# castorini/howl

Hardware: AMD Instinct MI355X
Metric: utterances/sec/node (res8 end-to-end training step, 1s@16kHz, 40-mel) (higher is better)
Workload: dtype f32; 1 GPU; res8 training step (frontend+fwd+xent+bwd+AdamW), 512 x 1 s utterances per GPU, 12 labels -- BASELINE configs[2] per-GPU share: res8 GSC-12, 512 x 1 s per GPU (4096 over 8); global_batch=512, samples_per_utterance=16000, labels=12, parallelism=single, frontend=eval

## Files before the change

### howl_amd/csrc/res8.hip

```cpp
#include "howl_common.hip.h"
#include "../../include/howl_hip.h"

namespace {

struct HowlPtrs6 {
    float* p[6];
};
constexpr int MAX_WINDOWS = 64;
struct HowlWinRows {
    int lo[MAX_WINDOWS], hi[MAX_WINDOWS];
};
struct HowlBnBuffers {
    float* running_mean;
    float* running_var;
    long long* num_batches;
};
struct BnFold {
    const float* part;
    int nparts;
    double count;
    float* stats_out;
    HowlBnBuffers bn;
};

// ... 631 lines not shown
#pragma unroll
                    for (int hh = 0; hh < 2; ++hh) ev[i][hh] = *reinterpret_cast<const float2*>(ebase + ea.off(i, hh));
            }
            HOWL_STAIR(1);
            k_run<NTW>(k, acc, c.CS, b2);
            k_tail<NTW>(k, acc, dl);
            HOWL_STAIR(0);
        }
        if constexpr (NTW > 0) conv_epilogue<MODE, NTW, TS, HALO>(acc, ev, epi, ubase, c.t0, lane, st0, st1, b, pv);
        __syncthreads();
    }
}

struct BwdFold {
    const float* stats;
    const float* m12;
    const float* part;
    int nparts;
    double count;
};
__device__ __forceinline__ void bwd_consts_to_lds(float* lm, int ch, float mean, float rstd, float m1, float m2) {
    lm[ch] = rstd;
    lm[CP + ch] = -rstd * rstd * m2;
    lm[2 * CP + ch] = rstd * (mean * rstd * m2 - m1);
}
__device__ __forceinline__ void bwd_fold_to_lds(float* lm, const BwdFold& f, int tid, int nthreads) {
    const int lane = tid & 63, wave = tid >> 6;
    if (f.part == nullptr) {
        if (tid < CP) bwd_consts_to_lds(lm, tid, f.stats[tid], f.stats[CP + tid], f.m12[tid], f.m12[CP + tid]);
    } else {
        const int c8 = lane >> 3;
        for (int ch0 = 4 * wave; ch0 < CP; ch0 += 4 * (nthreads >> 6)) {
            const int ch = ch0 + (c8 & 3);
            const float mean = f.stats[ch], rstd = f.stats[CP + ch];
            const double acc = fold_part_column(f.part, part_stride(f.nparts), f.nparts, (c8 < 4 ? 0 : CP) + ch, lane);
            const double second = __shfl_xor(acc, 32);
            if (c8 < 4 && (lane & 7) == 0)
                bwd_consts_to_lds(lm, ch, mean, rstd, (float)(acc / f.count), (float)(second / f.count));
        }
    }
}

struct WFold {
    const float* part;
    int nparts;
    float* out;
};

template <int MODE, int SLICES, int HALO = 0>
__device__ __forceinline__ void conv3x3_body(
    StageCfg cfg,
    const float* __restrict__ in_stats,
    const float* __restrict__ wp,
    const float* __restrict__ res,
// ... 741 lines not shown
        conv3x3_body<1, SD, HALO>(zc, nullptr, wp, nullptr, dx, xs, xs_stats, spart, nullptr, B, H, j, nblk, r, BnFold{}, bfold, wf, sg);
    else
        wgrad_body<SW, HALO>(WStage{zc, s_prev, false}, in_stats, bfold, wpart, B, H, j, nblk, r - SD, sg);
}

struct RowsAdamW {
    float* p;
    const float* g0;
    float* m;
    float* v;
    HowlAdamWCoef c;
    long rest_lo, rest_hi;
    int on;
};
__device__ __forceinline__ void reduce_rows_body(const float* __restrict__ part, int nparts, int ncols, int mode,
                                                 float* __restrict__ out, const RowsAdamW& opt) {
    __shared__ float red[16][64];
    const int lane = threadIdx.x & 63, rg = threadIdx.x >> 6, nrg = blockDim.x >> 6;
    const int col = blockIdx.x * 64 + lane;
    float s = 0.0f;
    if (col < ncols) {
        const float* src = part + col;
        for (int g = rg; g < nparts; g += 8 * nrg) {
            float v[8];
#pragma unroll
            for (int u = 0; u < 8; ++u) {
                const int r = g + u * nrg;
                v[u] = src[(size_t)(r < nparts ? r : nparts - 1) * ncols];
            }
#pragma unroll
            for (int u = 0; u < 8; ++u) s += (g + u * nrg < nparts) ? v[u] : 0.0f;
        }
    }
    red[rg][lane] = s;
    __syncthreads();
    if (rg == 0 && col < ncols) {
        float tot = red[0][lane];
        for (int r = 1; r < nrg; ++r) tot += red[r][lane];
        long d = -1;
        if (mode == 0) {
            d = col;
        } else {
            const int co = col / WNCOL, idx = col - co * WNCOL;
            if (co < NMAP && idx < WTAPS) d = (co * NMAP + idx % NMAP) * 9 + idx / NMAP;
        }
        if (d >= 0) {
            out[d] = tot;
            if (opt.on) howl_adamw_element(opt.p, opt.m, opt.v, (size_t)((out - opt.g0) + d), tot, opt.c);
        }
    }
}

__global__ __launch_bounds__(1024) void reduce_rows_all_kernel(const float* __restrict__ part, size_t layer_stride, int nparts,
                                                              HowlPtrs6 out, const float* __restrict__ c0part, int c0parts,
                                                              float* __restrict__ c0out, int y0, int yskip, int nrows, RowsAdamW opt) {
    if ((int)blockIdx.y >= nrows) {
        for (long i = opt.rest_lo + (long)blockIdx.x * blockDim.x + threadIdx.x; i < opt.rest_hi; i += (long)gridDim.x * blockDim.x)
            howl_adamw_element(opt.p, opt.m, opt.v, (size_t)i, opt.g0[i], opt.c);
        return;
    }
    const int y = y0 + (int)blockIdx.y * (1 + yskip);
    if (y < 6) {
        reduce_rows_body(part + y * layer_stride, nparts, CP * WNCOL, 1, out.p[y], opt);
    } else if (blockIdx.x * 64 < NMAP * 9) {
        reduce_rows_body(c0part, c0parts, NMAP * 9, 0, c0out, opt);
    }
}

__global__ void bn_eval_stats_kernel(HowlPtrs6 rmean, HowlPtrs6 rvar, float* __restrict__ stats) {
    const int layer = blockIdx.x, c = threadIdx.x;
    if (c >= CP) return;
    float* st = stats + (size_t)layer * 2 * CP;
    st[c] = (c < NMAP) ? rmean.p[layer][c] : 0.0f;
    st[CP + c] = (c < NMAP) ? 1.0f / sqrtf(rvar.p[layer][c] + BN_EPS) : 0.0f;
}

constexpr int BRB_THREADS = 1024;
__global__ __launch_bounds__(BRB_THREADS) void bn_relu_bwd_kernel(
    const float* __restrict__ dx,
    const float* __restrict__ dpool,
    const float* __restrict__ s, const float* __restrict__ stats, const float* __restrict__ m12,
    const float* __restrict__ part, int nparts, double count,
    const float* __restrict__ dskip,
    int even,
    float* __restrict__ ds_out,
    float* __restrict__ dz_out, int B, int P) {
    __shared__ float lm[4 * CP];
    const int tid = threadIdx.x, lane = tid & 63, wave = tid >> 6;
    if (tid < CP) {
        lm[tid] = stats[tid];
        lm[CP + tid] = stats[CP + tid];
        if (part == nullptr) {
            lm[2 * CP + tid] = m12[tid];
            lm[3 * CP + tid] = m12[CP + tid];
        }
    }
    if (part != nullptr) {
        const int c8 = lane >> 3;
        const int ch = 3 * wave + (c8 & 3);
        const bool used = (c8 & 3) < 3;
        const double acc = fold_part_column(part, part_stride(nparts), nparts, (c8 < 4 ? 0 : CP) + (used ? ch : 0), lane);
        const double second = __shfl_xor(acc, 32);
        if (c8 < 3 && (lane & 7) == 0) {
            lm[2 * CP + ch] = (float)(acc / count);
            lm[3 * CP + ch] = (float)(second / count);
        }
    }
    __syncthreads();
    const unsigned n2 = (unsigned)((size_t)B * NMAP * P / 2);
    const float invP = 1.0f / (float)P;
    const unsigned stride = gridDim.x * BRB_THREADS;
    auto finish = [&](float2 g, float2 sv, float2 kk, unsigned c, float2& ds, float2& dz) {
// ... 408 lines not shown
                    for (int i = rows.lo[w / ns] * PW + lane; i < rows.hi[w / ns] * PW; i += 64) acc += fabsf(src[i]);
                }
            }
            acc = wave_sum(acc);
            if (lane == 0) lp[c] = c < NMAP ? (acc * inv_count - stats[c]) * stats[CP + c] : 0.0f;
        }
        __syncthreads();
        for (int k = tid; k < C; k += 256) {
            float acc = bout[k];
            for (int c = 0; c < NMAP; ++c) acc = fmaf(wout[k * NMAP + c], lp[c], acc);
            logits[(size_t)b * C + k] = acc;
        }
    }
}

__global__ void head_bwd_pool_kernel(const float* __restrict__ dlogits, const float* __restrict__ wout,
                                     float* __restrict__ dpool, int B, int C) {
    const int idx = blockIdx.x * blockDim.x + threadIdx.x;
    if (idx >= B * CP) return;
    const int b = idx / CP, c = idx - b * CP;
    float acc = 0.0f;
    if (c < NMAP)
        for (int k = 0; k < C; ++k) acc = fmaf(dlogits[(size_t)b * C + k], wout[k * NMAP + c], acc);
    dpool[idx] = acc;
}

__global__ __launch_bounds__(1024) void head_bwd_param_kernel(const float* __restrict__ dlogits,
                                                              const float* __restrict__ pooled,
                                                              const float* __restrict__ dpool, float* __restrict__ dwout,
                                                              float* __restrict__ dbout, float* __restrict__ m12, int B,
                                                              int C, int P, const float* __restrict__ nll,
                                                              float* __restrict__ loss) {
    __shared__ double red[2][16][64];
    if ((int)blockIdx.x == C + 1) {
        double acc = 0.0;
        for (int b = threadIdx.x; b < B; b += 1024) acc += (double)nll[b];
        acc = wave_sum_d(acc);
        if ((threadIdx.x & 63) == 0) red[0][threadIdx.x >> 6][0] = acc;
        __syncthreads();
        if (threadIdx.x == 0) {
            double tot = 0.0;
            for (int w = 0; w < 16; ++w) tot += red[0][w][0];
            loss[0] = (float)(tot / (double)B);
        }
        return;
    }
    const int k = blockIdx.x, c = threadIdx.x & 63, bg = threadIdx.x >> 6;
    double a0 = 0.0, a1 = 0.0;
    constexpr int HR = 16;
    const int cc = c < CP ? c : CP - 1;
    if (k < C) {
        for (int b = bg; b < B; b += 16 * HR) {
            float d[HR], pv[HR];
#pragma unroll
            for (int j = 0; j < HR; ++j) {
                const int bb = b + 16 * j < B ? b + 16 * j : B - 1;
                d[j] = dlogits[(size_t)bb * C + k];
                pv[j] = pooled[(size_t)bb * CP + cc];
            }
#pragma unroll
            for (int j = 0; j < HR; ++j) {
// ... 20 lines not shown
        }
    }
    red[0][bg][c] = a0;
    red[1][bg][c] = a1;
    __syncthreads();
    if (bg != 0) return;
    double s0 = 0.0, s1 = 0.0;
    for (int g = 0; g < 16; ++g) {
        s0 += red[0][g][c];
        s1 += red[1][g][c];
    }
    if (k < C) {
        if (c < NMAP) dwout[k * NMAP + c] = (float)s0;
        if (c == 0) dbout[k] = (float)s1;
    } else if (c < CP) {
        const double n = (double)B * (double)P;
        m12[c] = (float)(s0 / n);
        m12[CP + c] = (float)(s1 / n);
    }
}

__global__ __launch_bounds__(1024) void xent_kernel(const float* __restrict__ logits, const long long* __restrict__ labels,
                                                    int B, int C, float* __restrict__ loss, float* __restrict__ dlogits) {
    __shared__ double red[16];
    double acc = 0.0;
    const float invB = 1.0f / (float)B;
    constexpr int XC = 32;
    for (int b = threadIdx.x; b < B; b += 1024) {
        const float* row = logits + (size_t)b * C;
        const int y = (int)labels[b];
        if (C <= XC) {
            float v[XC];
#pragma unroll
// ... 46 lines not shown

namespace {

size_t conv0_tile_floats(int T, int M) { return (size_t)(T + 2) * (M + 4) + 3 * (M + 4) + 16; }
size_t conv_lds_bytes(int H, bool own_rows) {
    return (size_t)(3 * KSTEPS * 64 + tile_floats(H, own_rows) + 4 * CP + 12 * 2 * 16) * sizeof(float);
}
size_t wgrad_lds_bytes(int H) { return (size_t)(tile_floats_z(H) + tile_floats_x(H) + 6 * CP) * sizeof(float); }

struct Ws {
    float* wp_fwd;
    float* wp_bwd;
    float* part;
    float* part2;
    float* stats;
    float* m12;
    float* dpool;
    float* pool;
    float* bufa;
    float* bufb;
    float* dz;
    float* dz2;
    float* dsa;
    float* dsb;
    float* wpart;
    float* c0part;
};

size_t ws_layout(Ws* w, char* base, int B, int H, int G, int cus, size_t* fwd_eval_bytes) {
    size_t off = 0;
    auto take = [&](size_t floats) {
        float* p = base ? reinterpret_cast<float*>(base + off) : nullptr;
        off += ((floats * sizeof(float) + 255) / 256) * 256;
        return p;
    };
    const size_t act = (size_t)B * NMAP * H * PW;
    w->wp_fwd = take((size_t)6 * 3 * KSTEPS * 64);
    w->wp_bwd = take((size_t)6 * 3 * KSTEPS * 64);
    const int max_parts = G > cus ? G : cus;
    w->part = take((size_t)part_stride(max_parts) * 2 * CP);
    w->part2 = take((size_t)part_stride(max_parts) * 2 * CP);
    w->stats = take((size_t)6 * 2 * CP);
    w->m12 = take(2 * CP);
    w->dpool = take((size_t)B * CP);
    w->pool = take((size_t)B * 16 * CP);
    *fwd_eval_bytes = off;
    w->bufa = take(act);
    w->bufb = take(act);
    w->dz = take(act);
    w->dz2 = take(act);
    w->dsa = take(act);
    w->dsb = take(act);
    w->wpart = take((size_t)6 * G * CP * WNCOL);
    w->c0part = take((size_t)max_parts * NMAP * 9);
    return off;
}

int mel_strips(int M) { return M == 40 ? 1 : (M == 80 ? 2 : 0); }
int even_grid(int g, int strips) { return strips > 1 ? ((g & ~1) > 2 ? (g & ~1) : 2) : g; }
int launch_blocks(int nblk, int per_group) { return 8 * per_group * ((nblk + 7) / 8); }
int conv_slices(int nblk, int H, int budget) {
    const int ntiles = (H * PW + 15) / 16;
    for (int sl = 4; sl > 1; sl >>= 1)
        if (nblk * sl <= budget && 4 * sl <= ntiles) return sl;
    return 1;
}
void pair_slices(int nblk, int H, int cus, int* sd, int* sw) {
    const int ntiles = (H * PW + 15) / 16;
    const int opts[3][2] = {{4, 2}, {2, 2}, {2, 1}};
// ... 289 lines not shown
        Conv3x3Launch a;
        a.in = plain_tile(sv->s[i - 1]);
        a.wp = w.wp_fwd + (size_t)(i - 1) * 3 * KSTEPS * 64;
        a.res = (i % 2) == 0 ? sv->s[i - 2] : nullptr;
        a.out = sv->s[i];
        a.part = training ? ((i & 1) ? w.part : w.part2) : nullptr;
        a.pool = i == 6 ? w.pool : nullptr;
        if (i > 1 && training)
            a.fold = fold_of(i - 1, (i & 1) ? w.part2 : w.part);
        else if (i > 1)
            a.in_stats = sv->bn_stats + (size_t)(i - 2) * 2 * CP;
        HowlProfScope prof("conv3x3_fwd", stream);
        launch_conv3x3<0>(p, stream, a);
    }
    const int groups = 4 * p.SL;
    hipLaunchKernelGGL(head_fwd_kernel, dim3(B < 1024 ? B : 1024), dim3(HEAD_THREADS), 0, stream, sv->s[6],
                       sv->bn_stats + (size_t)5 * 2 * CP, prm->out_w, prm->out_b, sv->pooled, logits, B, p.Pt, C, labels, nll, dlogits,
                       w.dpool, 1.0f / (float)B, (const float*)w.pool, groups, groups < (p.P + 15) / 16 ? groups : (p.P + 15) / 16,
                       training ? fold_of(6, w.part2) : BnFold{}, p.nr * p.ns);
    HOWL_CHECK_LAUNCH("howl_res8_fwd");
    return HOWL_OK;
}

int res8_bwd_impl(const HowlRes8Params* prm, const Feat& feat, int B, int T, int M, int C, const HowlRes8Saved* sv, const float* dlogits,
                  const HowlRes8Grads* gr, void* ws, size_t ws_bytes, int part, const float* nll, float* loss, hipStream_t stream,
                  const HowlAdamW* adamw = nullptr) {
    HOWL_REQUIRE(prm && feat.x && sv && dlogits && gr && ws, "howl_res8_bwd: null pointer");
    HOWL_REQUIRE(adamw == nullptr || (part == 0 && adamw->p && adamw->g && adamw->m && adamw->v && adamw->n >= 1 && adamw->step >= 1),
                 "howl_res8_bwd: HowlAdamW needs the whole pass (part 0) and complete buffers");
    HOWL_REQUIRE(part >= 0 && part <= 2, "howl_res8_bwd_part: part must be 0 (all), 1 or 2");
    const bool run_layers = part != 2, run_conv0 = part != 1;
    HOWL_REQUIRE(mel_strips(M) > 0, "howl_res8_bwd: M must be 40 or 80 (got %d)", M);
    HOWL_REQUIRE(B >= 1 && T / 3 >= 1, "howl_res8_bwd: B=%d T=%d unsupported", B, T);
    const Res8Plan p = res8_plan(B, T, M, ws);
    HOWL_REQUIRE(p.hv_last >= 1 && p.nr <= MAX_ROW_STRIPS, "howl_res8_bwd: T=%d frames unsupported (%d row strips)", T, p.nr);
    if (int rc = check_workspace("howl_res8_bwd", ws_bytes, p.train_bytes)) return rc;
    HOWL_REQUIRE(p.saved_floats / 2 < (size_t)1 << 31, "howl_res8_bwd: B=%d too large for the 32-bit element index of the elementwise pass", B);
    const Ws& w = p.ws;
    const double count = (double)B * (double)p.Pt;

    if (run_layers) {
        if (nll == nullptr)
            hipLaunchKernelGGL(head_bwd_pool_kernel, dim3((B * CP + 255) / 256), dim3(256), 0, stream, dlogits, prm->out_w, w.dpool,
                               B, C);
        hipLaunchKernelGGL(head_bwd_param_kernel, dim3(C + (nll != nullptr ? 2 : 1)), dim3(1024), 0, stream, dlogits, sv->pooled,
                           w.dpool, gr->out_w, gr->out_b, w.m12, B, C, p.Pt, nll, loss);
    }
    float* dx_cur = nullptr;
    float* dx_next = w.bufa;
    float* ds_prev = nullptr;
    float* ds_free = w.dsa;
    for (int i = 6; i >= 1; --i) {
        const bool even = (i % 2) == 0;
        const float* stats_i = sv->bn_stats + (size_t)(i - 1) * 2 * CP;
        float* ds_out = even ? ds_free : nullptr;
        float* dz = even ? w.dz : w.dz2;
        float* part_in = p.fused ? ((i & 1) ? w.part2 : w.part) : w.part;
        float* part_out = p.fused ? ((i & 1) ? w.part : w.part2) : w.part;
        BwdLayerLaunch a;
        a.bfold = BwdFold{stats_i, w.m12, i == 6 ? (const float*)nullptr : (const float*)part_in, p.Gh * p.SD, count};
        a.zc = plain_tile(dz);
        if (p.fused)
            a.zc = StageCfg{dx_cur, sv->s[i], even ? (const float*)ds_prev : (const float*)nullptr, ds_out, w.dpool,
                            1.0f / (float)p.Pt, true, even, false};
        else if (run_layers)
            hipLaunchKernelGGL(bn_relu_bwd_kernel, dim3(p.ew_grid), dim3(BRB_THREADS), 0, stream, (const float*)dx_cur, w.dpool, sv->s[i],
                               stats_i, w.m12, a.bfold.part, p.Gh * p.SD, count, even ? (const float*)ds_prev : (const float*)nullptr,
                               even ? 1 : 0, ds_out, dz, B, p.P);
        if (even) {
            float* t = ds_prev ? ds_prev : w.dsb;
            ds_prev = ds_out;
            ds_free = t;
        }
        const bool need_stats = i > 1;
        a.s_prev = sv->s[i - 1];
        a.in_stats = need_stats ? sv->bn_stats + (size_t)(i - 2) * 2 * CP : nullptr;
        a.wp = w.wp_bwd + (size_t)(i - 1) * 3 * KSTEPS * 64;
        a.dx = dx_next;
        a.xs = need_stats ? sv->s[i - 1] : (const float*)ds_prev;
        a.xs_stats = a.in_stats;
        a.spart = need_stats ? part_out : nullptr;
        a.wpart = w.wpart + (size_t)(i - 1) * p.wpart_stride;
// ... 7 lines not shown
                HowlProfScope prof("conv3x3_dgrad", stream);
                Conv3x3Launch d;
                d.in = a.zc, d.wp = a.wp, d.out = a.dx, d.xs = a.xs, d.xs_stats = a.xs_stats, d.part = a.spart;
                d.bfold = a.bfold, d.wf = a.wf;
                launch_conv3x3<1>(p, stream, d);
            }
            HowlProfScope prof("wgrad", stream);
            launch_wgrad(p, stream, a);
        }
        dx_cur = dx_next;
        dx_next = (dx_next == w.bufa) ? w.bufb : w.bufa;
    }
    HOWL_REQUIRE(sv->mask0 != nullptr, "howl_res8_bwd: saved->mask0 is required");
    const HowlPtrs6 gw = ptrs6(gr->conv_w);
    const RowsAdamW no_opt{nullptr, nullptr, nullptr, nullptr, HowlAdamWCoef{}, 0, 0, 0};
    const auto reduce_rows = [&](int cols, int first, int skip, int nrows, const RowsAdamW& opt) {
        hipLaunchKernelGGL(reduce_rows_all_kernel, dim3((cols + 63) / 64, nrows + (opt.on ? 1 : 0)), dim3(1024), 0, stream,
                           (const float*)w.wpart, p.wpart_stride, p.Gh, gw, (const float*)w.c0part, p.G0w, gr->conv0_w, first, skip,
                           nrows, opt);
    };
    if (part == 1)
        reduce_rows(CP * WNCOL, 0, 0, p.fold_in_pair ? 1 : 6, no_opt);
    if (run_conv0) {
        {
            HowlProfScope prof("conv0_wgrad", stream);
            launch_conv0_wgrad(p, stream, feat, sv->mask0, dx_cur);
        }
        if (part == 0) {
            RowsAdamW opt = no_opt;
            bool own_launch = adamw != nullptr;
            if (adamw != nullptr && getenv("HOWL_NO_FOLD_ADAMW") == nullptr) {
                const float* g0 = adamw->g;
                bool flat = gr->conv0_w == g0 && gr->out_b == gr->out_w + (size_t)NMAP * C &&
                            adamw->n == (size_t)NMAP * 9 + (size_t)6 * NMAP * NMAP * 9 + (size_t)NMAP * C + (size_t)C &&
                            gr->out_w == g0 + (size_t)NMAP * 9 + (size_t)6 * NMAP * NMAP * 9;
                for (int i = 0; i < 6; ++i) flat = flat && gr->conv_w[i] == g0 + (size_t)NMAP * 9 + (size_t)i * NMAP * NMAP * 9;
                if (flat) {
                    opt = RowsAdamW{adamw->p, g0, adamw->m, adamw->v,
                                    howl_adamw_coef(adamw->lr, adamw->beta1, adamw->beta2, adamw->eps, adamw->weight_decay, adamw->step,
                                                    adamw->grad_scale),
                                    (long)((p.fold_in_pair ? gr->conv_w[1] : gr->out_w) - g0), (long)adamw->n, 1};
                    own_launch = false;
                }
            }
            reduce_rows(CP * WNCOL, 0, p.fold_in_pair ? 5 : 0, p.fold_in_pair ? 2 : 7, opt);
            if (own_launch) {
                const int rc = howl_adamw_step(adamw->p, adamw->g, adamw->m, adamw->v, adamw->n, adamw->lr, adamw->beta1, adamw->beta2,
                                               adamw->eps, adamw->weight_decay, adamw->step, adamw->grad_scale, stream);
                if (rc != HOWL_OK) return rc;
            }
        } else {
            reduce_rows(NMAP * 9, 6, 0, 1, no_opt);
        }
    }
    HOWL_CHECK_LAUNCH("howl_res8_bwd");
    return HOWL_OK;
}

}

extern "C" {

size_t howl_res8_workspace_bytes(int B, int T) { return res8_plan(B, T, 40).train_bytes; }
size_t howl_res8_workspace_bytes_mels(int B, int T, int M) { return res8_plan(B, T, M).train_bytes; }
size_t howl_res8_saved_floats(int B, int T, int M) { return res8_plan(B, T, M).saved_floats; }
size_t howl_res8_eval_workspace_bytes_mels(int B, int T, int M) { return res8_plan(B, T, M).eval_bytes; }
int howl_res8_row_strips(int T) { return res8_plan(1, T, 40).nr; }

int howl_res8_fwd(const HowlRes8Params* prm, const float* feat, long sb, long st, long sm, int B, int T, int M, int C,
                  int training, const HowlRes8Saved* sv, float* logits, void* ws, size_t ws_bytes, hipStream_t stream) {
    return res8_fwd_impl(prm, Feat{feat, sb, st, sm}, B, T, M, C, training, sv, logits, ws, ws_bytes, nullptr, nullptr, nullptr, stream);
}

size_t howl_res8_long_workspace_bytes(int B, int T) { return res8_long_plan(B, T, 40).long_bytes; }
size_t howl_res8_long_workspace_bytes_mels(int B, int T, int M) { return res8_long_plan(B, T, M).long_bytes; }

int howl_res8_fwd_long(const HowlRes8Params* prm, const float* feat, long sb, long st, long sm, int B, int T, int M, int C,
                       float* logits, void* ws, size_t ws_bytes, hipStream_t stream) {
    HOWL_REQUIRE(prm && feat && logits && ws, "howl_res8_fwd_long: null pointer");
    HOWL_REQUIRE(mel_strips(M) > 0, "howl_res8_fwd_long: res8 pools (3,4) over 40 or 80 mel bins; got M=%d", M);
    const int H = T / 3;
    HOWL_REQUIRE(B >= 1 && H > WIN_H && C >= 1, "howl_res8_fwd_long: for T > 83 frames (got B=%d T=%d); shorter inputs use howl_res8_fwd", B, T);
// ... 91 lines not shown
```

### howl_amd/lib.py

```python
import ctypes
import os
from ctypes import POINTER, c_char_p, c_double, c_float, c_int, c_long, c_size_t, c_void_p
from pathlib import Path

LIB_PATH = Path(os.environ.get("HOWL_HIP_LIBRARY") or Path(__file__).resolve().parent / "libhowl_hip.so")
MAX_MELS = 96
FB_COLS = 48
FB_PACKED_FLOATS = 260 * FB_COLS + 17 * 64 * 4 + 17 * (FB_COLS // 4) * 64 + 32


def fb_packed_floats(n_mels: int) -> int:
    return FB_PACKED_FLOATS * (1 if n_mels <= FB_COLS else 2)


P = c_void_p
STREAM = c_void_p


class HowlMelPoints(ctypes.Structure):
    _fields_ = [("f", c_float * (MAX_MELS + 2))]


class HowlRes8Params(ctypes.Structure):
    _fields_ = [("conv0_w", P), ("conv_w", P * 6), ("bn_running_mean", P * 6), ("bn_running_var", P * 6),
# ... 41 lines not shown
class HowlLstmSaved(ctypes.Structure):
    _fields_ = [("gx", P), ("gates", P), ("c", P), ("hseq", P), ("dgates", P), ("t_out", c_int), ("x_frames", c_int)]


class HowlMbLayer(ctypes.Structure):
    _fields_ = [(n, c_int) for n in ("kind", "cin", "cout", "stride", "pad_h", "pad_w", "act", "bias", "pool", "res_src",
                                     "feat", "sub", "wrapped")] + \
               [(n, ctypes.c_longlong) for n in ("w_off", "b_off", "gamma_off", "beta_off", "rmean_off", "rvar_off")]


class HowlMbWsLayer(ctypes.Structure):
    _fields_ = [(n, ctypes.c_longlong) for n in ("z", "g", "y", "ss", "bc", "b_ss", "f_yout", "pooled", "pooled_d", "dz1",
                                                 "total_floats")] + \
               [(n, c_int) for n in ("hin", "win", "ho", "wo", "hy", "wy", "f_tile", "f_cx", "f_ry", "d_tile", "d_ry", "d_chunks",
                                     "nslab", "group_rows")]


class HowlDecideConfig(ctypes.Structure):
    _fields_ = [("mode", c_int), ("C", c_int), ("blank", c_int), ("negative", c_int), ("threshold", c_double), ("smoothing_ms", c_double),
                ("window_ms", c_double), ("tolerance_ms", c_double), ("seq_len", c_int), ("sequence", c_int * 16), ("weights", P),
                ("color", P)]


SIGNATURES = {
    "howl_version": [POINTER(c_int), POINTER(c_int)],
    "howl_profile_enable": [c_int],
    "howl_profile_read": [c_char_p, POINTER(c_double), POINTER(c_int), c_int],
    "howl_profile_read_work": [c_char_p, POINTER(c_double), POINTER(c_int), POINTER(c_double), c_int],
    "howl_shutdown": [],
    "howl_fb_pack": [P, c_int, P, STREAM],
# ... 37 lines not shown
    "howl_seq_head_ctc": [POINTER(HowlHeadParams), P, c_long, c_long, c_int, c_int, c_int, c_int, c_int, P, c_long, c_int, P, P, c_int, P, P,
                          P, P, P, c_size_t, STREAM],
    "howl_seq_head_ctc_supported": [c_int, c_int, c_int, c_int, c_int, c_int],
    "howl_seq_lstm_bwd": [POINTER(HowlHeadParams), c_int, c_int, P, P, P, P, POINTER(HowlHeadGrads), POINTER(HowlCtcMean), P,
                          c_size_t, POINTER(HowlLstmParams), P, c_int, c_int, c_int, P, P, POINTER(HowlLstmSaved),
                          POINTER(HowlLstmGrads), P, c_size_t, POINTER(HowlAdamW), STREAM],
    "howl_adamw_step": [P, P, P, P, c_size_t, c_float, c_float, c_float, c_float, c_float, c_int, c_float, STREAM],
    "howl_mobilenet_layer": [c_int, POINTER(HowlMbLayer)],
    "howl_mobilenet_workspace_layer": [c_int, c_int, c_int, c_int, c_int, POINTER(HowlMbWsLayer)],
    "howl_mobilenet_fwd": [P, P, c_int, P, c_long, c_long, c_long, c_int, c_int, c_int, c_int, P, c_float, P, P, c_size_t,
                           STREAM],
    "howl_mobilenet_bwd": [P, c_int, P, c_long, c_long, c_long, c_int, c_int, c_int, P, c_float, P, P, P, c_size_t, STREAM],
}
SIZE_FUNCS = {"howl_fb_packed_floats": [c_int], "howl_res8_workspace_bytes": [c_int, c_int], "howl_res8_long_workspace_bytes": [c_int, c_int],
              "howl_res8_workspace_bytes_mels": [c_int, c_int, c_int], "howl_res8_saved_floats": [c_int, c_int, c_int],
              "howl_res8_eval_workspace_bytes_mels": [c_int, c_int, c_int], "howl_res8_row_strips": [c_int], "howl_res8_long_workspace_bytes_mels": [c_int, c_int, c_int], "howl_lstm_workspace_bytes": [c_int, c_int],
              "howl_lstm_needs_gx": [POINTER(HowlLstmParams), c_int, c_int, c_int, c_int],
              "howl_head_workspace_bytes": [c_int, c_int, c_int],
              "howl_mobilenet_num_layers": [],
              "howl_mobilenet_param_floats": [c_int], "howl_mobilenet_buffer_floats": [],
              "howl_mobilenet_workspace_bytes": [c_int, c_int, c_int, c_int],
              "howl_ctc_supported": [c_int, c_int, c_int], "howl_ctc_workspace_floats": [c_int, c_int]}


STREAM_SIGNATURES = {
    "howl_res8_stream_prepare": [POINTER(HowlRes8Params), c_int, P, c_size_t, STREAM],
    "howl_res8_stream_windows": [P, P, c_long, c_int, c_int, P, c_int, c_float, P, c_int, P, P, STREAM],
}
STREAM_SIZE_FUNCS = {"howl_res8_stream_supported": [c_int, c_int, c_int], "howl_res8_stream_state_bytes": [c_int]}

LSTM_STREAM_SIGNATURES = {
# ... 52 lines not shown
```

### include/howl_hip.h

```cpp
#ifndef HOWL_HIP_H
#define HOWL_HIP_H

#include <stddef.h>
#include <stdint.h>

#ifdef __cplusplus
extern "C" {
#endif

typedef struct ihipStream_t* hipStream_t;

#define HOWL_FB_COLS 48
#define HOWL_MAX_MELS 96
#define HOWL_FB_PACKED_FLOATS (260 * HOWL_FB_COLS + 17 * 64 * 4 + 17 * (HOWL_FB_COLS / 4) * 64 + 32)

int howl_version(int* major, int* minor);
const char* howl_last_error(void);

int howl_profile_enable(int on);
int howl_profile_read(const char* tag, double* total_ms, int* count, int reset);
int howl_profile_read_work(const char* tag, double* total_ms, int* count, double* work, int reset);

int howl_shutdown(void);

// ... 55 lines not shown
    float* out_b;
} HowlRes8Grads;

typedef struct {
    float* s[7];
    float* bn_stats;
    float* pooled;
    unsigned short* mask0;
} HowlRes8Saved;

size_t howl_res8_workspace_bytes(int B, int T);
size_t howl_res8_workspace_bytes_mels(int B, int T, int M);
size_t howl_res8_saved_floats(int B, int T, int M);
size_t howl_res8_eval_workspace_bytes_mels(int B, int T, int M);
int howl_res8_row_strips(int T);

int howl_res8_fwd(const HowlRes8Params* prm, const float* feat, long sb, long st, long sm, int B, int T, int M, int C,
                  int training, const HowlRes8Saved* saved, float* logits, void* ws, size_t ws_bytes,
                  hipStream_t stream);

size_t howl_res8_long_workspace_bytes(int B, int T);
size_t howl_res8_long_workspace_bytes_mels(int B, int T, int M);
int howl_res8_fwd_long(const HowlRes8Params* prm, const float* feat, long sb, long st, long sm, int B, int T, int M, int C,
                       float* logits, void* ws, size_t ws_bytes, hipStream_t stream);

int howl_res8_bwd(const HowlRes8Params* prm, const float* feat, long sb, long st, long sm, int B, int T, int M, int C,
                  const HowlRes8Saved* saved, const float* dlogits, const HowlRes8Grads* grads, void* ws,
                  size_t ws_bytes, hipStream_t stream);
int howl_res8_bwd_part(const HowlRes8Params* prm, const float* feat, long sb, long st, long sm, int B, int T, int M, int C,
                       const HowlRes8Saved* saved, const float* dlogits, const HowlRes8Grads* grads, void* ws,
// ... 153 lines not shown
```

Before: 463,200 utterances/sec.

## Group head xent/backward per utterance block and fold partials into row reduction

Replaces the per-utterance head forward plus separate head backward parameter kernel with a grouped kernel that computes pooled BN, logits, cross-entropy, dlogits and dpool for a block of utterances. Each block writes per-group partial sums for the head weight gradients and the BN backward moments. Those partials are then reduced inside the existing reduce_rows launch, which also takes over the loss mean and applies AdamW to the head parameters. The m12 buffer is removed and BN backward always folds the partials. The aim is to cut small serial head launches and the C+1-block parameter kernel, at the cost of an extra partial buffer and a coupled launch structure.

```diff
diff --git a/howl_amd/csrc/res8.hip b/howl_amd/csrc/res8.hip
--- a/howl_amd/csrc/res8.hip
+++ b/howl_amd/csrc/res8.hip
@@ -669,7 +669,6 @@
 
 struct BwdFold {
     const float* stats;
-    const float* m12;
     const float* part;
     int nparts;
     double count;
@@ -681,18 +680,14 @@
 }
 __device__ __forceinline__ void bwd_fold_to_lds(float* lm, const BwdFold& f, int tid, int nthreads) {
     const int lane = tid & 63, wave = tid >> 6;
-    if (f.part == nullptr) {
-        if (tid < CP) bwd_consts_to_lds(lm, tid, f.stats[tid], f.stats[CP + tid], f.m12[tid], f.m12[CP + tid]);
-    } else {
-        const int c8 = lane >> 3;
-        for (int ch0 = 4 * wave; ch0 < CP; ch0 += 4 * (nthreads >> 6)) {
-            const int ch = ch0 + (c8 & 3);
-            const float mean = f.stats[ch], rstd = f.stats[CP + ch];
-            const double acc = fold_part_column(f.part, part_stride(f.nparts), f.nparts, (c8 < 4 ? 0 : CP) + ch, lane);
-            const double second = __shfl_xor(acc, 32);
-            if (c8 < 4 && (lane & 7) == 0)
-                bwd_consts_to_lds(lm, ch, mean, rstd, (float)(acc / f.count), (float)(second / f.count));
-        }
+    const int c8 = lane >> 3;
+    for (int ch0 = 4 * wave; ch0 < CP; ch0 += 4 * (nthreads >> 6)) {
+        const int ch = ch0 + (c8 & 3);
+        const float mean = f.stats[ch], rstd = f.stats[CP + ch];
+        const double acc = fold_part_column(f.part, part_stride(f.nparts), f.nparts, (c8 < 4 ? 0 : CP) + ch, lane);
+        const double second = __shfl_xor(acc, 32);
+        if (c8 < 4 && (lane & 7) == 0)
+            bwd_consts_to_lds(lm, ch, mean, rstd, (float)(acc / f.count), (float)(second / f.count));
     }
 }
 
@@ -1464,7 +1459,8 @@
     int on;
 };
 __device__ __forceinline__ void reduce_rows_body(const float* __restrict__ part, int nparts, int ncols, int mode,
-                                                 float* __restrict__ out, const RowsAdamW& opt) {
+                                                 float* __restrict__ out, const RowsAdamW& opt, float* __restrict__ out_hi = nullptr,
+                                                 int split = 0) {
     __shared__ float red[16][64];
     const int lane = threadIdx.x & 63, rg = threadIdx.x >> 6, nrg = blockDim.x >> 6;
     const int col = blockIdx.x * 64 + lane;
@@ -1487,24 +1483,58 @@
     if (rg == 0 && col < ncols) {
         float tot = red[0][lane];
         for (int r = 1; r < nrg; ++r) tot += red[r][lane];
-        long d = -1;
+        float* dst = nullptr;
         if (mode == 0) {
-            d = col;
+            dst = (out_hi != nullptr && col >= split) ? out_hi + (col - split) : out + col;
         } else {
             const int co = col / WNCOL, idx = col - co * WNCOL;
-            if (co < NMAP && idx < WTAPS) d = (co * NMAP + idx % NMAP) * 9 + idx / NMAP;
-        }
-        if (d >= 0) {
-            out[d] = tot;
-            if (opt.on) howl_adamw_element(opt.p, opt.m, opt.v, (size_t)((out - opt.g0) + d), tot, opt.c);
-        }
+            if (co < NMAP && idx < WTAPS) dst = out + (co * NMAP + idx % NMAP) * 9 + idx / NMAP;
+        }
+        if (dst != nullptr) {
+            *dst = tot;
+            if (opt.on) howl_adamw_element(opt.p, opt.m, opt.v, (size_t)(dst - opt.g0), tot, opt.c);
+        }
+    }
+}
+
+struct HeadRows {
+    const float* part;
+    int nparts, C;
+    float* out_w;
+    float* out_b;
+    const float* nll;
+    float* loss;
+    int B;
+};
+__device__ __forceinline__ void loss_mean_body(const float* __restrict__ nll, int B, float* __restrict__ loss) {
+    __shared__ double red[16];
+    double acc = 0.0;
+    for (int b = threadIdx.x; b < B; b += 1024) acc += (double)nll[b];
+    acc = wave_sum_d(acc);
+    if ((threadIdx.x & 63) == 0) red[threadIdx.x >> 6] = acc;
+    __syncthreads();
+    if (threadIdx.x == 0) {
+        double tot = 0.0;
+        for (int w = 0; w < 16; ++w) tot += red[w];
+        loss[0] = (float)(tot / (double)B);
     }
 }
 
 __global__ __launch_bounds__(1024) void reduce_rows_all_kernel(const float* __restrict__ part, size_t layer_stride, int nparts,
                                                               HowlPtrs6 out, const float* __restrict__ c0part, int c0parts,
-                                                              float* __restrict__ c0out, int y0, int yskip, int nrows, RowsAdamW opt) {
-    if ((int)blockIdx.y >= nrows) {
+                                                              float* __restrict__ c0out, int y0, int yskip, int nrows, HeadRows head,
+                                                              RowsAdamW opt) {
+    int extra = (int)blockIdx.y - nrows;
+    if (extra >= 0) {
+        if (head.part != nullptr && extra-- == 0) {
+            const int ncols = head.C * NMAP + head.C;
+            if ((int)blockIdx.x * 64 < ncols) reduce_rows_body(head.part, head.nparts, ncols, 0, head.out_w, opt, head.out_b, head.C * NMAP);
+            return;
+        }
+        if (head.nll != nullptr && extra-- == 0) {
+            if (blockIdx.x == 0) loss_mean_body(head.nll, head.B, head.loss);
+            return;
+        }
         for (long i = opt.rest_lo + (long)blockIdx.x * blockDim.x + threadIdx.x; i < opt.rest_hi; i += (long)gridDim.x * blockDim.x)
             howl_adamw_element(opt.p, opt.m, opt.v, (size_t)i, opt.g0[i], opt.c);
         return;
@@ -1529,7 +1559,7 @@
 __global__ __launch_bounds__(BRB_THREADS) void bn_relu_bwd_kernel(
     const float* __restrict__ dx,
     const float* __restrict__ dpool,
-    const float* __restrict__ s, const float* __restrict__ stats, const float* __restrict__ m12,
+    const float* __restrict__ s, const float* __restrict__ stats,
     const float* __restrict__ part, int nparts, double count,
     const float* __restrict__ dskip,
     int even,
@@ -1540,12 +1570,8 @@
     if (tid < CP) {
         lm[tid] = stats[tid];
         lm[CP + tid] = stats[CP + tid];
-        if (part == nullptr) {
-            lm[2 * CP + tid] = m12[tid];
-            lm[3 * CP + tid] = m12[CP + tid];
-        }
-    }
-    if (part != nullptr) {
+    }
+    {
         const int c8 = lane >> 3;
         const int ch = 3 * wave + (c8 & 3);
         const bool used = (c8 & 3) < 3;
@@ -1984,6 +2010,150 @@
     }
 }
 
+constexpr int HEAD_U = HEAD_THREADS / 64;
+__device__ __forceinline__ void head_group_rows(const float (*pl)[CP], const float (*dl)[HEAD_XC], const float (*dp)[CP], int nu,
+                                                int group, int ngroups, int C, float* __restrict__ part, float* __restrict__ hpart) {
+    const int tid = threadIdx.x;
+    if (tid < CP) {
+        double a0 = 0.0, a1 = 0.0;
+        for (int u = 0; u < nu; ++u) {
+            a0 += (double)dp[u][tid];
+            a1 = fma((double)dp[u][tid], (double)pl[u][tid], a1);
+        }
+        const int nps = part_stride(ngroups);
+        part[(size_t)tid * nps + group] = (float)a0;
+        part[(size_t)(CP + tid) * nps + group] = (float)a1;
+    }
+    const int nw = C * NMAP;
+    float* row = hpart + (size_t)group * (nw + C);
+    for (int i = tid; i < nw + C; i += HEAD_THREADS) {
+        float acc = 0.0f;
+        if (i < nw) {
+            const int k = i / NMAP, c = i - k * NMAP;
+            for (int u = 0; u < nu; ++u) acc = fmaf(dl[u][k], pl[u][c], acc);
+        } else {
+            for (int u = 0; u < nu; ++u) acc += dl[u][i - nw];
+        }
+        row[i] = acc;
+    }
+}
+__device__ __forceinline__ void head_wave_dpool(const float* dl, const float* lw, int C, int lane, float* dp, float* __restrict__ dpool_b) {
+    if (lane < CP) {
+        float acc = 0.0f;
+        if (lane < NMAP)
+            for (int k = 0; k < C; ++k) acc = fmaf(dl[k], lw[k * NMAP + lane], acc);
+        dp[lane] = acc;
+        dpool_b[lane] = acc;
+    }
+}
+
+__global__ __launch_bounds__(HEAD_THREADS) void head_xent_group_kernel(
+    const float* __restrict__ wout, const float* __restrict__ bout, float* __restrict__ pooled, float* __restrict__ logits, int B, int P,
+    int C, const long long* __restrict__ labels, float* __restrict__ nll, float* __restrict__ dlogits, float* __restrict__ dpool,
+    float inv_batch, const float* __restrict__ pool, int npg, int npg_used, BnFold fold,
+    int ns , float* __restrict__ part_out,
+    float* __restrict__ hpart) {
+    __shared__ float lst[2 * CP];
+    __shared__ float lw[HEAD_XC * NMAP];
+    __shared__ float pl[HEAD_U][CP], dp[HEAD_U][CP], ll[HEAD_U][HEAD_XC], dl[HEAD_U][HEAD_XC];
+    const int tid = threadIdx.x, lane = tid & 63, wave = tid >> 6;
+    for (int i = tid; i < C * NMAP; i += HEAD_THREADS) lw[i] = wout[i];
+    {
+        const int c8 = lane >> 3;
+        for (int w0 = wave; w0 < CP / 4; w0 += HEAD_U) {
+            const int c = 4 * w0 + (c8 & 3);
+            const double sm = fold_part_column(fold.part, part_stride(fold.nparts), fold.nparts, (c8 < 4 ? 0 : CP) + c, lane);
+            const double q = __shfl_xor(sm, 32);
+            if (c8 < 4 && (lane & 7) == 0) {
+                const double mean = sm / fold.count;
+                double var = q / fold.count - mean * mean;
+                var = var < 0.0 ? 0.0 : var;
+                const float fm = (c < NMAP) ? (float)mean : 0.0f;
+                const float fr = (c < NMAP) ? (float)(1.0 / sqrt(var + (double)BN_EPS)) : 0.0f;
+                lst[c] = fm;
+                lst[CP + c] = fr;
+                if (blockIdx.x == 0) {
+                    fold.stats_out[c] = fm;
+                    fold.stats_out[CP + c] = fr;
+                    if (c < NMAP && fold.bn.running_mean != nullptr) {
+                        const double unbiased = fold.count > 1.0 ? var * fold.count / (fold.count - 1.0) : var;
+                        fold.bn.running_mean[c] = (1.0f - BN_MOMENTUM) * fold.bn.running_mean[c] + BN_MOMENTUM * (float)mean;
+                        fold.bn.running_var[c] = (1.0f - BN_MOMENTUM) * fold.bn.running_var[c] + BN_MOMENTUM * (float)unbiased;
+                    }
+                    if (c == 0 && fold.bn.num_batches != nullptr) fold.bn.num_batches[0] += 1;
+                }
+            }
+        }
+    }
+    __syncthreads();
+    const int group = blockIdx.x, b = group * HEAD_U + wave;
+    if (b < B) {
+        const int nparts = ns * npg_used;
+        const int pc = lane < CP ? lane : CP - 1;
+        float acc = 0.0f;
+        for (int k0 = 0; k0 < nparts; k0 += 16) {
+            float v[16];
+#pragma unroll
+            for (int j = 0; j < 16; ++j) {
+                const int k = k0 + j < nparts ? k0 + j : nparts - 1;
+                const int sgi = k / npg_used, g = k - sgi * npg_used;
+                v[j] = pool[(((size_t)b * ns + sgi) * npg + g) * CP + pc];
+            }
+#pragma unroll
+            for (int j = 0; j < 16; ++j) acc = (k0 + j < nparts) ? acc + v[j] : acc;
+        }
+        if (lane < CP) {
+            const float v = lane < NMAP ? (acc / (float)P - lst[lane]) * lst[CP + lane] : 0.0f;
+            pl[wave][lane] = v;
+            pooled[(size_t)b * CP + lane] = v;
+        }
+        wave_lds_sync();
+        if (lane < C) {
+            float lg = bout[lane];
+            for (int c = 0; c < NMAP; ++c) lg = fmaf(lw[lane * NMAP + c], pl[wave][c], lg);
+            logits[(size_t)b * C + lane] = lg;
+            ll[wave][lane] = lg;
+        }
+        wave_lds_sync();
+        const int y = (int)labels[b];
+        float mx = ll[wave][0];
+        for (int k = 1; k < C; ++k) mx = fmaxf(mx, ll[wave][k]);
+        float se = 0.0f;
+        for (int k = 0; k < C; ++k) se += expf(ll[wave][k] - mx);
+        const float lse = mx + logf(se);
+        if (lane == 0) nll[b] = lse - ll[wave][y];
+        if (lane < C) {
+            const float d = (expf(ll[wave][lane] - lse) - (lane == y ? 1.0f : 0.0f)) * inv_batch;
+            dl[wave][lane] = d;
+            dlogits[(size_t)b * C + lane] = d;
+        }
+        wave_lds_sync();
+        head_wave_dpool(dl[wave], lw, C, lane, dp[wave], dpool + (size_t)b * CP);
+    }
+    __syncthreads();
+    const int left = B - group * HEAD_U;
+    head_group_rows(pl, dl, dp, left < HEAD_U ? left : HEAD_U, group, gridDim.x, C, part_out, hpart);
+}
+
+__global__ __launch_bounds__(HEAD_THREADS) void head_bwd_group_kernel(const float* __restrict__ dlogits, const float* __restrict__ wout,
+                                                                      const float* __restrict__ pooled, float* __restrict__ dpool, int B,
+                                                                      int C, float* __restrict__ part_out, float* __restrict__ hpart) {
+    __shared__ float lw[HEAD_XC * NMAP];
+    __shared__ float pl[HEAD_U][CP], dp[HEAD_U][CP], dl[HEAD_U][HEAD_XC];
+    const int tid = threadIdx.x, lane = tid & 63, wave = tid >> 6;
+    for (int i = tid; i < C * NMAP; i += HEAD_THREADS) lw[i] = wout[i];
+    const int group = blockIdx.x, b = group * HEAD_U + wave;
+    if (b < B) {
+        if (lane < CP) pl[wave][lane] = pooled[(size_t)b * CP + lane];
+        if (lane < C) dl[wave][lane] = dlogits[(size_t)b * C + lane];
+    }
+    __syncthreads();
+    if (b < B) head_wave_dpool(dl[wave], lw, C, lane, dp[wave], dpool + (size_t)b * CP);
+    __syncthreads();
+    const int left = B - group * HEAD_U;
+    head_group_rows(pl, dl, dp, left < HEAD_U ? left : HEAD_U, group, gridDim.x, C, part_out, hpart);
+}
+
 __global__ void head_bwd_pool_kernel(const float* __restrict__ dlogits, const float* __restrict__ wout,
                                      float* __restrict__ dpool, int B, int C) {
     const int idx = blockIdx.x * blockDim.x + threadIdx.x;
@@ -1998,23 +2168,9 @@
 __global__ __launch_bounds__(1024) void head_bwd_param_kernel(const float* __restrict__ dlogits,
                                                               const float* __restrict__ pooled,
                                                               const float* __restrict__ dpool, float* __restrict__ dwout,
-                                                              float* __restrict__ dbout, float* __restrict__ m12, int B,
-                                                              int C, int P, const float* __restrict__ nll,
-                                                              float* __restrict__ loss) {
+                                                              float* __restrict__ dbout, float* __restrict__ part, int B,
+                                                              int C) {
     __shared__ double red[2][16][64];
-    if ((int)blockIdx.x == C + 1) {
-        double acc = 0.0;
-        for (int b = threadIdx.x; b < B; b += 1024) acc += (double)nll[b];
-        acc = wave_sum_d(acc);
-        if ((threadIdx.x & 63) == 0) red[0][threadIdx.x >> 6][0] = acc;
-        __syncthreads();
-        if (threadIdx.x == 0) {
-            double tot = 0.0;
-            for (int w = 0; w < 16; ++w) tot += red[0][w][0];
-            loss[0] = (float)(tot / (double)B);
-        }
-        return;
-    }
     const int k = blockIdx.x, c = threadIdx.x & 63, bg = threadIdx.x >> 6;
     double a0 = 0.0, a1 = 0.0;
     constexpr int HR = 16;
@@ -2065,9 +2221,8 @@
         if (c < NMAP) dwout[k * NMAP + c] = (float)s0;
         if (c == 0) dbout[k] = (float)s1;
     } else if (c < CP) {
-        const double n = (double)B * (double)P;
-        m12[c] = (float)(s0 / n);
-        m12[CP + c] = (float)(s1 / n);
+        part[(size_t)c * part_stride(1)] = (float)s0;
+        part[(size_t)(CP + c) * part_stride(1)] = (float)s1;
     }
 }
 
@@ -2144,7 +2299,6 @@
     float* part;
     float* part2;
     float* stats;
-    float* m12;
     float* dpool;
     float* pool;
     float* bufa;
@@ -2155,7 +2309,9 @@
     float* dsb;
     float* wpart;
     float* c0part;
-};
+    float* hpart;
+};
+int head_groups(int B) { return (B + HEAD_U - 1) / HEAD_U; }
 
 size_t ws_layout(Ws* w, char* base, int B, int H, int G, int cus, size_t* fwd_eval_bytes) {
     size_t off = 0;
@@ -2167,11 +2323,11 @@
     const size_t act = (size_t)B * NMAP * H * PW;
     w->wp_fwd = take((size_t)6 * 3 * KSTEPS * 64);
     w->wp_bwd = take((size_t)6 * 3 * KSTEPS * 64);
-    const int max_parts = G > cus ? G : cus;
+    int max_parts = G > cus ? G : cus;
+    if (head_groups(B) > max_parts) max_parts = head_groups(B);
     w->part = take((size_t)part_stride(max_parts) * 2 * CP);
     w->part2 = take((size_t)part_stride(max_parts) * 2 * CP);
     w->stats = take((size_t)6 * 2 * CP);
-    w->m12 = take(2 * CP);
     w->dpool = take((size_t)B * CP);
     w->pool = take((size_t)B * 16 * CP);
     *fwd_eval_bytes = off;
@@ -2183,6 +2339,7 @@
     w->dsb = take(act);
     w->wpart = take((size_t)6 * G * CP * WNCOL);
     w->c0part = take((size_t)max_parts * NMAP * 9);
+    w->hpart = take((size_t)head_groups(B) * HEAD_XC * (NMAP + 1));
     return off;
 }
 
@@ -2502,10 +2659,15 @@
         launch_conv3x3<0>(p, stream, a);
     }
     const int groups = 4 * p.SL;
-    hipLaunchKernelGGL(head_fwd_kernel, dim3(B < 1024 ? B : 1024), dim3(HEAD_THREADS), 0, stream, sv->s[6],
-                       sv->bn_stats + (size_t)5 * 2 * CP, prm->out_w, prm->out_b, sv->pooled, logits, B, p.Pt, C, labels, nll, dlogits,
-                       w.dpool, 1.0f / (float)B, (const float*)w.pool, groups, groups < (p.P + 15) / 16 ? groups : (p.P + 15) / 16,
-                       training ? fold_of(6, w.part2) : BnFold{}, p.nr * p.ns);
+    if (labels != nullptr)
+        hipLaunchKernelGGL(head_xent_group_kernel, dim3(head_groups(B)), dim3(HEAD_THREADS), 0, stream, prm->out_w, prm->out_b, sv->pooled,
+                           logits, B, p.Pt, C, labels, nll, dlogits, w.dpool, 1.0f / (float)B, (const float*)w.pool, groups,
+                           groups < (p.P + 15) / 16 ? groups : (p.P + 15) / 16, fold_of(6, w.part2), p.nr * p.ns, w.part, w.hpart);
+    else
+        hipLaunchKernelGGL(head_fwd_kernel, dim3(B < 1024 ? B : 1024), dim3(HEAD_THREADS), 0, stream, sv->s[6],
+                           sv->bn_stats + (size_t)5 * 2 * CP, prm->out_w, prm->out_b, sv->pooled, logits, B, p.Pt, C, labels, nll, dlogits,
+                           w.dpool, 1.0f / (float)B, (const float*)w.pool, groups, groups < (p.P + 15) / 16 ? groups : (p.P + 15) / 16,
+                           training ? fold_of(6, w.part2) : BnFold{}, p.nr * p.ns);
     HOWL_CHECK_LAUNCH("howl_res8_fwd");
     return HOWL_OK;
 }
@@ -2517,6 +2679,7 @@
     HOWL_REQUIRE(adamw == nullptr || (part == 0 && adamw->p && adamw->g && adamw->m && adamw->v && adamw->n >= 1 && adamw->step >= 1),
                  "howl_res8_bwd: HowlAdamW needs the whole pass (part 0) and complete buffers");
     HOWL_REQUIRE(part >= 0 && part <= 2, "howl_res8_bwd_part: part must be 0 (all), 1 or 2");
+    HOWL_REQUIRE(nll == nullptr || C <= HEAD_XC, "howl_res8_bwd_xent: follows howl_res8_fwd_xent, at most %d classes (C=%d)", HEAD_XC, C);
     const bool run_layers = part != 2, run_conv0 = part != 1;
     HOWL_REQUIRE(mel_strips(M) > 0, "howl_res8_bwd: M must be 40 or 80 (got %d)", M);
     HOWL_REQUIRE(B >= 1 && T / 3 >= 1, "howl_res8_bwd: B=%d T=%d unsupported", B, T);
@@ -2527,13 +2690,21 @@
     const Ws& w = p.ws;
     const double count = (double)B * (double)p.Pt;
 
-    if (run_layers) {
-        if (nll == nullptr)
+    const bool grouped = C <= HEAD_XC;
+    const int head_rows = grouped ? head_groups(B) : 1;
+    if (run_layers && nll == nullptr) {
+        if (grouped) {
+            hipLaunchKernelGGL(head_bwd_group_kernel, dim3(head_groups(B)), dim3(HEAD_THREADS), 0, stream, dlogits, prm->out_w,
+                               (const float*)sv->pooled, w.dpool, B, C, w.part, w.hpart);
+        } else {
             hipLaunchKernelGGL(head_bwd_pool_kernel, dim3((B * CP + 255) / 256), dim3(256), 0, stream, dlogits, prm->out_w, w.dpool,
                                B, C);
-        hipLaunchKernelGGL(head_bwd_param_kernel, dim3(C + (nll != nullptr ? 2 : 1)), dim3(1024), 0, stream, dlogits, sv->pooled,
-                           w.dpool, gr->out_w, gr->out_b, w.m12, B, C, p.Pt, nll, loss);
-    }
+            hipLaunchKernelGGL(head_bwd_param_kernel, dim3(C + 1), dim3(1024), 0, stream, dlogits, (const float*)sv->pooled,
+                               (const float*)w.dpool, gr->out_w, gr->out_b, w.part, B, C);
+        }
+    }
+    const HeadRows head{grouped ? (const float*)w.hpart : (const float*)nullptr, head_groups(B), C, gr->out_w, gr->out_b, nll, loss, B};
+    const HeadRows no_head{nullptr, 0, 0, nullptr, nullptr, nullptr, nullptr, 0};
     float* dx_cur = nullptr;
     float* dx_next = w.bufa;
     float* ds_prev = nullptr;
@@ -2546,14 +2717,14 @@
         float* part_in = p.fused ? ((i & 1) ? w.part2 : w.part) : w.part;
         float* part_out = p.fused ? ((i & 1) ? w.part : w.part2) : w.part;
         BwdLayerLaunch a;
-        a.bfold = BwdFold{stats_i, w.m12, i == 6 ? (const float*)nullptr : (const float*)part_in, p.Gh * p.SD, count};
+        a.bfold = BwdFold{stats_i, part_in, i == 6 ? head_rows : p.Gh * p.SD, count};
         a.zc = plain_tile(dz);
         if (p.fused)
             a.zc = StageCfg{dx_cur, sv->s[i], even ? (const float*)ds_prev : (const float*)nullptr, ds_out, w.dpool,
                             1.0f / (float)p.Pt, true, even, false};
         else if (run_layers)
             hipLaunchKernelGGL(bn_relu_bwd_kernel, dim3(p.ew_grid), dim3(BRB_THREADS), 0, stream, (const float*)dx_cur, w.dpool, sv->s[i],
-                               stats_i, w.m12, a.bfold.part, p.Gh * p.SD, count, even ? (const float*)ds_prev : (const float*)nullptr,
+                               stats_i, a.bfold.part, a.bfold.nparts, count, even ? (const float*)ds_prev : (const float*)nullptr,
                                even ? 1 : 0, ds_out, dz, B, p.P);
         if (even) {
             float* t = ds_prev ? ds_prev : w.dsb;
@@ -2591,13 +2762,14 @@
     HOWL_REQUIRE(sv->mask0 != nullptr, "howl_res8_bwd: saved->mask0 is required");
     const HowlPtrs6 gw = ptrs6(gr->conv_w);
     const RowsAdamW no_opt{nullptr, nullptr, nullptr, nullptr, HowlAdamWCoef{}, 0, 0, 0};
-    const auto reduce_rows = [&](int cols, int first, int skip, int nrows, const RowsAdamW& opt) {
-        hipLaunchKernelGGL(reduce_rows_all_kernel, dim3((cols + 63) / 64, nrows + (opt.on ? 1 : 0)), dim3(1024), 0, stream,
+    const auto reduce_rows = [&](int cols, int first, int skip, int nrows, const HeadRows& hd, const RowsAdamW& opt) {
+        const int extra = (hd.part != nullptr ? 1 : 0) + (hd.nll != nullptr ? 1 : 0) + (opt.on ? 1 : 0);
+        hipLaunchKernelGGL(reduce_rows_all_kernel, dim3((cols + 63) / 64, nrows + extra), dim3(1024), 0, stream,
                            (const float*)w.wpart, p.wpart_stride, p.Gh, gw, (const float*)w.c0part, p.G0w, gr->conv0_w, first, skip,
-                           nrows, opt);
+                           nrows, hd, opt);
     };
     if (part == 1)
-        reduce_rows(CP * WNCOL, 0, 0, p.fold_in_pair ? 1 : 6, no_opt);
+        reduce_rows(CP * WNCOL, 0, 0, p.fold_in_pair ? 1 : 6, head, no_opt);
     if (run_conv0) {
         {
             HowlProfScope prof("conv0_wgrad", stream);
@@ -2616,18 +2788,18 @@
                     opt = RowsAdamW{adamw->p, g0, adamw->m, adamw->v,
                                     howl_adamw_coef(adamw->lr, adamw->beta1, adamw->beta2, adamw->eps, adamw->weight_decay, adamw->step,
                                                     adamw->grad_scale),
-                                    (long)((p.fold_in_pair ? gr->conv_w[1] : gr->out_w) - g0), (long)adamw->n, 1};
+                                    (long)((p.fold_in_pair ? gr->conv_w[1] : gr->out_w) - g0), (long)(gr->out_w - g0), 1};
                     own_launch = false;
                 }
             }
-            reduce_rows(CP * WNCOL, 0, p.fold_in_pair ? 5 : 0, p.fold_in_pair ? 2 : 7, opt);
+            reduce_rows(CP * WNCOL, 0, p.fold_in_pair ? 5 : 0, p.fold_in_pair ? 2 : 7, head, opt);
             if (own_launch) {
                 const int rc = howl_adamw_step(adamw->p, adamw->g, adamw->m, adamw->v, adamw->n, adamw->lr, adamw->beta1, adamw->beta2,
                                                adamw->eps, adamw->weight_decay, adamw->step, adamw->grad_scale, stream);
                 if (rc != HOWL_OK) return rc;
             }
         } else {
-            reduce_rows(NMAP * 9, 6, 0, 1, no_opt);
+            reduce_rows(NMAP * 9, 6, 0, 1, no_head, no_opt);
         }
     }
     HOWL_CHECK_LAUNCH("howl_res8_bwd");
@@ -2643,6 +2815,28 @@
 size_t howl_res8_saved_floats(int B, int T, int M) { return res8_plan(B, T, M).saved_floats; }
 size_t howl_res8_eval_workspace_bytes_mels(int B, int T, int M) { return res8_plan(B, T, M).eval_bytes; }
 int howl_res8_row_strips(int T) { return res8_plan(1, T, 40).nr; }
+
+size_t howl_res8_workspace_head(int B, int T, int M, int C, HowlRes8WsHead* out) {
+    if (out == nullptr || mel_strips(M) == 0 || B < 1 || T / 3 < 1 || C < 1) {
+        howl_set_error("howl_res8_workspace_head: null pointer or bad shape (B=%d T=%d M=%d C=%d)", B, T, M, C);
+        return 0;
+    }
+    char* const base = reinterpret_cast<char*>(256);
+    const Res8Plan p = res8_plan(B, T, M, base);
+    const auto at = [&](const float* q) { return (long long)((reinterpret_cast<const char*>(q) - base) / (long)sizeof(float)); };
+    const bool grouped = C <= HEAD_XC;
+    HowlRes8WsHead o{};
+    o.dpool = at(p.ws.dpool);
+    o.sums = at(p.ws.part);
+    o.grads = at(p.ws.hpart);
+    o.group_utterances = grouped ? HEAD_U : B;
+    o.sums_rows = grouped ? head_groups(B) : 1;
+    o.sums_stride = part_stride(o.sums_rows);
+    o.grad_rows = grouped ? head_groups(B) : 0;
+    o.grad_width = grouped ? C * NMAP + C : 0;
+    *out = o;
+    return p.train_bytes;
+}
 
 int howl_res8_fwd(const HowlRes8Params* prm, const float* feat, long sb, long st, long sm, int B, int T, int M, int C,
                   int training, const HowlRes8Saved* sv, float* logits, void* ws, size_t ws_bytes, hipStream_t stream) {
diff --git a/howl_amd/lib.py b/howl_amd/lib.py
--- a/howl_amd/lib.py
+++ b/howl_amd/lib.py
@@ -79,6 +79,11 @@
                                                  "total_floats")] + \
                [(n, c_int) for n in ("hin", "win", "ho", "wo", "hy", "wy", "f_tile", "f_cx", "f_ry", "d_tile", "d_ry", "d_chunks",
                                      "nslab", "group_rows")]
+
+
+class HowlRes8WsHead(ctypes.Structure):
+    _fields_ = [(n, ctypes.c_longlong) for n in ("dpool", "sums", "grads")] + \
+               [(n, c_int) for n in ("group_utterances", "sums_rows", "sums_stride", "grad_rows", "grad_width")]
 
 
 class HowlDecideConfig(ctypes.Structure):
@@ -146,7 +151,8 @@
 }
 SIZE_FUNCS = {"howl_fb_packed_floats": [c_int], "howl_res8_workspace_bytes": [c_int, c_int], "howl_res8_long_workspace_bytes": [c_int, c_int],
               "howl_res8_workspace_bytes_mels": [c_int, c_int, c_int], "howl_res8_saved_floats": [c_int, c_int, c_int],
-              "howl_res8_eval_workspace_bytes_mels": [c_int, c_int, c_int], "howl_res8_row_strips": [c_int], "howl_res8_long_workspace_bytes_mels": [c_int, c_int, c_int], "howl_lstm_workspace_bytes": [c_int, c_int],
+              "howl_res8_eval_workspace_bytes_mels": [c_int, c_int, c_int],
+              "howl_res8_workspace_head": [c_int, c_int, c_int, c_int, POINTER(HowlRes8WsHead)], "howl_res8_row_strips": [c_int], "howl_res8_long_workspace_bytes_mels": [c_int, c_int, c_int], "howl_lstm_workspace_bytes": [c_int, c_int],
               "howl_lstm_needs_gx": [POINTER(HowlLstmParams), c_int, c_int, c_int, c_int],
               "howl_head_workspace_bytes": [c_int, c_int, c_int],
               "howl_mobilenet_num_layers": [],
diff --git a/include/howl_hip.h b/include/howl_hip.h
--- a/include/howl_hip.h
+++ b/include/howl_hip.h
@@ -93,6 +93,11 @@
 size_t howl_res8_saved_floats(int B, int T, int M);
 size_t howl_res8_eval_workspace_bytes_mels(int B, int T, int M);
 int howl_res8_row_strips(int T);
+typedef struct {
+    long long dpool, sums, grads;
+    int group_utterances, sums_rows, sums_stride, grad_rows, grad_width;
+} HowlRes8WsHead;
+size_t howl_res8_workspace_head(int B, int T, int M, int C, HowlRes8WsHead* out);
 
 int howl_res8_fwd(const HowlRes8Params* prm, const float* feat, long sb, long st, long sm, int B, int T, int M, int C,
                   int training, const HowlRes8Saved* saved, float* logits, void* ws, size_t ws_bytes,
```

After: 467,800 utterances/sec (median of 6 runs). Within noise of the previous version (+1.0%).
